# NVlabs/FoundationPose

Hardware: NVIDIA H100
Metric: pose-hypotheses/sec at 640x480 RGB-D, 252 hyp, 5 refine iters (higher is better)
Workload: dtype f16

## Files before the change

foundationpose_b200/csrc/fp_api_ops.cu:

```cuda
#include "../../include/fpose.h"
#include "fp_common.cuh"
#include "fp_attn.cuh"
#include "fp_crop.cuh"
#include "fp_gemm.cuh"

#include <vector>

namespace fp {
const char* get_last_error();
int prof_collect(int kind, double* total_ms, double* total_work, int* launches);
int pose_errors_launch(const float* pts, int P, const float* pred, int N, const float* gt, int n_gt, float* add_out,
                       float* adds_out, cudaStream_t stream);
int sym_pose_errors_launch(const float* pts, int P, const float* pred, int N, const float* gt, int n_gt, const float* sym,
                           int S, const float* K, int n_K, float* mssd_out, float* mspd_out, cudaStream_t stream);
}

static int check_device_ptr(const void* p, const char* what, const char* fn = "fp_pose_errors") {
  int dev = 0;
  FP_CUDA_OK(cudaGetDevice(&dev));
  cudaPointerAttributes a;
  const cudaError_t e = cudaPointerGetAttributes(&a, p);
  if (e != cudaSuccess) {
    cudaGetLastError();
    fp::set_last_error("%s: %s: cudaPointerGetAttributes failed (%s)", fn, what, cudaGetErrorString(e));
// ... 43 lines not shown
      }
    std::vector<float> nrm((size_t)V * 3, 0.f), att((size_t)V * 3, 0.f);
    fp::MeshHost mh;
    int rc = fp::build_mesh_host(V, F, pos, nrm.data(), att.data(), 3, faces, mh);
    if (rc) return rc;
    int max_t = 0, max_v = 0, total = 0;
    for (const fp::Meshlet& m : mh.meshlets) {
      max_t = m.n_tris > max_t ? m.n_tris : max_t;
      max_v = m.n_verts > max_v ? m.n_verts : max_v;
      total += m.n_tris;
      for (int t = 0; t < m.n_tris; ++t) {
        const uint2 tr = mh.ml_tris[m.tri_off + t];
        for (int k = 0; k < 3; ++k) {
          const int slot = (tr.x >> (8 * k)) & 255;
          if (slot >= m.n_verts || mh.ml_verts[m.vert_off + slot] != faces[3 * tr.y + k]) {
            fp::set_last_error("fp_op_build_meshlets: meshlet triangle does not map back to its face");
            return -4;
          }
          const float* q = pos + 3 * faces[3 * tr.y + k];
          const float dx = q[0] - m.cx, dy = q[1] - m.cy, dz = q[2] - m.cz;
          if (dx * dx + dy * dy + dz * dz > m.r * m.r * 1.0001f + 1e-12f) {
            fp::set_last_error("fp_op_build_meshlets: vertex outside the meshlet's bounding sphere");
            return -4;
          }
        }
        if (face_of_tri_out) face_of_tri_out[m.tri_off + t] = (int)tr.y;
      }
    }
    if (meshlets_out)
      for (size_t i = 0; i < mh.meshlets.size(); ++i) {
        const fp::Meshlet& m = mh.meshlets[i];
        const float rec[8] = {m.cx, m.cy, m.cz, m.r, m.ax, m.ay, m.az, m.cutoff};
        for (int k = 0; k < 8; ++k) meshlets_out[8 * i + k] = rec[k];
      }
    info[0] = (int)mh.meshlets.size();
    info[1] = mh.closed;
    info[2] = mh.front_sign;
    info[3] = max_t;
    info[4] = max_v;
    info[5] = total;
    return 0;
  } catch (...) {
    fp::set_last_error("fp_op_build_meshlets: exception");
    return -3;
  }
}

int fp_op_attention(const void* qkv, void* out, int B, int impl, void* stream) {
  if (!qkv || !out) {
    fp::set_last_error("fp_op_attention: null argument");
    return -1;
  }
  (void)impl;
  return fp::attn_tc_launch(
      fp::head_attn_params(reinterpret_cast<const __half*>(qkv), 1536, 1, reinterpret_cast<__half*>(out), B),
      reinterpret_cast<cudaStream_t>(stream));
}

static int check_dev16(const void* p, const char* what, const char* fn) {
  FP_REQUIRE(p, "%s: %s is null", fn, what);
  FP_REQUIRE(reinterpret_cast<uintptr_t>(p) % 16 == 0, "%s: %s is not 16-byte aligned", fn, what);
  return check_device_ptr(p, what, fn);
}

int fp_op_attention_groups(const void* qkv, int ld, int n_groups, void* out, int B, void* stream) {
  const char* fn = "fp_op_attention_groups";
  FP_REQUIRE(n_groups == 1 || n_groups == 2, "%s: n_groups = %d, must be 1 or 2", fn, n_groups);
  FP_REQUIRE(ld >= 1536 * n_groups && ld % 8 == 0, "%s: ld = %d, must be a multiple of 8 and >= %d", fn, ld, 1536 * n_groups);
  FP_REQUIRE(B >= 0 && B <= FP_OP_MAX_SEQUENCES, "%s: B = %d outside [0, %d]", fn, B, FP_OP_MAX_SEQUENCES);
  if (check_dev16(qkv, "qkv", fn) || check_dev16(out, "out", fn)) return -1;
  return fp::attn_core_launch(
      fp::head_attn_params(reinterpret_cast<const __half*>(qkv), ld, n_groups, reinterpret_cast<__half*>(out), B),
      reinterpret_cast<cudaStream_t>(stream));
}

int fp_op_layernorm(const void* x, void* y, const float* gamma, const float* beta, int rows, void* stream) {
  const char* fn = "fp_op_layernorm";
  FP_REQUIRE(rows >= 0 && rows <= FP_OP_MAX_SEQUENCES * 400, "%s: rows = %d outside [0, %d]", fn, rows,
             FP_OP_MAX_SEQUENCES * 400);
  if (check_dev16(x, "x", fn) || check_dev16(y, "y", fn) || check_dev16(gamma, "gamma", fn) || check_dev16(beta, "beta", fn))
    return -1;
  return fp::layernorm_launch(reinterpret_cast<const __half*>(x), reinterpret_cast<__half*>(y), gamma, beta, rows,
                              reinterpret_cast<cudaStream_t>(stream));
}

int fp_op_head_final(const void* x, const float* gamma, const float* beta, const float* w, const float* bias, float* out,
                     int B, int out_dim, void* stream) {
  const char* fn = "fp_op_head_final";
  FP_REQUIRE(B >= 0 && B <= FP_OP_MAX_SEQUENCES, "%s: B = %d outside [0, %d]", fn, B, FP_OP_MAX_SEQUENCES);
  FP_REQUIRE(out_dim >= 1 && out_dim <= 8, "%s: out_dim = %d outside [1, 8]", fn, out_dim);
  if (check_dev16(x, "x", fn) || check_dev16(gamma, "gamma", fn) || check_dev16(beta, "beta", fn)) return -1;
  FP_REQUIRE(w && bias && out, "%s: null w, bias or out", fn);
  if (check_device_ptr(w, "w", fn) || check_device_ptr(bias, "bias", fn) || check_device_ptr(out, "out", fn)) return -1;
  return fp::head_final_launch(reinterpret_cast<const __half*>(x), gamma, beta, w, bias, out, B, 400, out_dim,
                               reinterpret_cast<cudaStream_t>(stream));
}

int fp_op_token_mean_proj(const void* x, const float* w_f32, const float* bias, float* mean_ws, float* out, int B,
                          void* stream) {
  const char* fn = "fp_op_token_mean_proj";
  FP_REQUIRE(B >= 0 && B <= FP_OP_MAX_SEQUENCES, "%s: B = %d outside [0, %d]", fn, B, FP_OP_MAX_SEQUENCES);
  if (check_dev16(x, "x", fn) || check_dev16(w_f32, "w_f32", fn) || check_dev16(mean_ws, "mean_ws", fn)) return -1;
  FP_REQUIRE(bias && out, "%s: null bias or out", fn);
  if (check_device_ptr(bias, "bias", fn) || check_device_ptr(out, "out", fn)) return -1;
  return fp::token_mean_proj_launch(reinterpret_cast<const __half*>(x), w_f32, bias, mean_ws, out, B, 400,
                                    reinterpret_cast<cudaStream_t>(stream));
}

static fp::GemmLayer to_gemm_layer(const fp_gemm_layer_t* l) {
  fp::GemmLayer L;
  L.kind = l->kind;
  L.n_img = l->n_img;
  L.Hin = l->Hin;
  L.Win = l->Win;
  L.Cin = l->Cin;
  L.Cout = l->Cout;
  L.in = l->in;
  L.w = l->w;
  L.bias = l->bias;
  L.res = l->res;
  L.res_ld = l->res_ld;
  L.out = l->out;
  L.out_ld = l->out_ld;
  L.out_split = l->out_split;
  L.post_add = l->post_add;
  L.relu = l->relu;
  return L;
}

int fp_op_gemm_layer(const fp_gemm_layer_t* l, void* stream) {
  if (!l) {
    fp::set_last_error("fp_op_gemm_layer: null layer");
    return -1;
  }
  return fp::gemm_layer_launch(to_gemm_layer(l), reinterpret_cast<cudaStream_t>(stream));
}

int fp_op_gemm_tile_n(const fp_gemm_layer_t* l, int* tile_n) {
  if (!l || !tile_n) {
    fp::set_last_error("fp_op_gemm_tile_n: null argument");
    return -1;
  }
  return fp::gemm_layer_tile_n(to_gemm_layer(l), tile_n);
}

int fp_op_gemm_tile_m(const fp_gemm_layer_t* l, int* tile_m) {
  if (!l || !tile_m) {
    fp::set_last_error("fp_op_gemm_tile_m: null argument");
    return -1;
  }
  return fp::gemm_layer_tile_m(to_gemm_layer(l), tile_m);
}

int fp_pose_errors(const float* pts, int P, const float* pred, int N, const float* gt, int n_gt, float* add_out,
                   float* adds_out, void* stream) {
  FP_REQUIRE(P >= 1 && P <= FP_METRICS_MAX_POINTS, "fp_pose_errors: P = %d outside [1, %d]", P, FP_METRICS_MAX_POINTS);
  FP_REQUIRE(N >= 0 && N <= FP_METRICS_MAX_POSES, "fp_pose_errors: N = %d outside [0, %d]", N, FP_METRICS_MAX_POSES);
  FP_REQUIRE(n_gt == 1 || n_gt == N, "fp_pose_errors: n_gt = %d, must be 1 or N = %d", n_gt, N);
  if (N == 0) return 0;
  FP_REQUIRE(pts && pred && gt, "fp_pose_errors: null input pointer");
  const void* ptrs[5] = {pts, pred, gt, add_out, adds_out};
  const char* names[5] = {"pts", "pred", "gt", "add_out", "adds_out"};
  for (int i = 0; i < 5; ++i)
    if (ptrs[i] && check_device_ptr(ptrs[i], names[i])) return -1;
  return fp::pose_errors_launch(pts, P, pred, N, gt, n_gt, add_out, adds_out, reinterpret_cast<cudaStream_t>(stream));
}

int fp_sym_pose_errors(const float* pts, int P, const float* pred, int N, const float* gt, int n_gt, const float* sym,
                       int S, const float* K, int n_K, float* mssd_out, float* mspd_out, void* stream) {
  FP_REQUIRE(P >= 1 && P <= FP_METRICS_MAX_POINTS, "fp_sym_pose_errors: P = %d outside [1, %d]", P, FP_METRICS_MAX_POINTS);
  FP_REQUIRE(N >= 0 && N <= FP_METRICS_MAX_POSES, "fp_sym_pose_errors: N = %d outside [0, %d]", N, FP_METRICS_MAX_POSES);
  FP_REQUIRE(S >= 1 && S <= FP_METRICS_MAX_SYMMETRIES, "fp_sym_pose_errors: S = %d outside [1, %d]", S,
             FP_METRICS_MAX_SYMMETRIES);
  FP_REQUIRE(n_gt == 1 || n_gt == N, "fp_sym_pose_errors: n_gt = %d, must be 1 or N = %d", n_gt, N);
  if (mspd_out) FP_REQUIRE(n_K == 1 || n_K == N, "fp_sym_pose_errors: n_K = %d, must be 1 or N = %d", n_K, N);
  if (N == 0) return 0;
  FP_REQUIRE(pts && pred && gt && sym, "fp_sym_pose_errors: null input pointer");
  FP_REQUIRE(K || !mspd_out, "fp_sym_pose_errors: mspd_out needs K");
  const void* ptrs[7] = {pts, pred, gt, sym, mspd_out ? K : nullptr, mssd_out, mspd_out};
  const char* names[7] = {"pts", "pred", "gt", "sym", "K", "mssd_out", "mspd_out"};
  for (int i = 0; i < 7; ++i)
    if (ptrs[i] && check_device_ptr(ptrs[i], names[i], "fp_sym_pose_errors")) return -1;
  return fp::sym_pose_errors_launch(pts, P, pred, N, gt, n_gt, sym, S, K, n_K, mssd_out, mspd_out,
                                    reinterpret_cast<cudaStream_t>(stream));
}

}
```

foundationpose_b200/csrc/fp_gemm.cu:

```cuda
#include "fp_gemm.cuh"

#include <stdarg.h>
#include <stdlib.h>
#include <string.h>

#include <mutex>
#include <vector>

#include "fp_common.cuh"
#include "fp_wgmma.cuh"

namespace fp {

static std::atomic<unsigned long long> g_launch_count{0};
static thread_local bool t_capturing = false;
void note_launches(int n) {
  if (!t_capturing) g_launch_count.fetch_add((unsigned long long)n, std::memory_order_relaxed);
}
unsigned long long launch_count() { return g_launch_count.load(std::memory_order_relaxed); }
void set_capturing(bool on) { t_capturing = on; }

std::atomic<bool> g_prof_on{false};
static std::mutex g_prof_mu;

// ... 252 lines not shown
        mbar_arrive(&empty[prev]);
      }
      prev = stage;
      if (++stage == S) {
        stage = 0;
        phase ^= 1;
      }
    }
    if constexpr (kSwap) {
      const float bc[2] = {__ldg(p.bias + n_tile * BN + r0), __ldg(p.bias + n_tile * BN + r0 + 8)};
      wgmma_wait<0>();
      fence_regs(acc);
      if (prev >= 0) mbar_arrive(&empty[prev]);
      if (p.has_res) mbar_wait(&res_full[0], (uint32_t)(it & 1));
      else asm volatile("bar.sync 1, 256;" ::: "memory");
      const int mi = lane >> 3, mr = lane & 7;
      const uint32_t lane_off =
          (uint32_t)(8 * (mi >> 1) + mr) * 128u + ((uint32_t)((2 * ((ct >> 5) & 3) + (mi & 1)) ^ mr) << 4);
#pragma unroll
      for (int ph = 0; ph < 2; ++ph) {
        const uint32_t slab = smem_u32(staging + (2 * ph + cw) * kSlabBytes) + lane_off;
        uint32_t rv[8][4];
        if (p.has_res) {
#pragma unroll
          for (int g = 0; g < 8; ++g) ldsm_x4_trans(slab + g * 2048u, rv[g]);
        }
#pragma unroll
        for (int g = 0; g < 8; ++g) {
          uint32_t o[4];
#pragma unroll
          for (int i = 0; i < 4; ++i) {
            const int j = 16 * ph + 2 * g + (i >> 1), h = i & 1;
            float a0 = acc[4 * j + 2 * h] + bc[h], a1 = acc[4 * j + 2 * h + 1] + bc[h];
            if (p.has_res) {
              const float2 r = __half22float2(*reinterpret_cast<const __half2*>(&rv[g][i]));
              a0 += r.x;
              a1 += r.y;
            }
            if (p.relu) {
              a0 = fmaxf(a0, 0.f);
              a1 = fmaxf(a1, 0.f);
            }
            o[i] = pack_half2(a0, a1);
          }
          stsm_x4_trans(slab + g * 2048u, o);
        }
      }
      asm volatile("fence.proxy.async.shared::cta;" ::: "memory");
      asm volatile("bar.sync 1, 256;" ::: "memory");
      if (leader) {
        for (int q = 0; q < NSLAB; ++q)
          tma_store_5d(&map_out, staging + q * kSlabBytes, coff + n_tile * BN + slab_ch(q), oc[1], oc[2],
                       oc[3] + slab_img(q), oc[4]);
        asm volatile("cp.async.bulk.commit_group;" ::: "memory");
      }
      continue;
    }
    const float* bias = p.bias + n_tile * BN;
    const float* pap[2] = {nullptr, nullptr};
    if (p.post_add) {
#pragma unroll
      for (int h = 0; h < 2; ++h) {
        const int row = r0 + 8 * h;
        const int jj = row & (p.bw - 1), ii = (row >> p.lg_bw) & (p.bh - 1);
        const int i = th * p.bh + ii, j = min(tw * p.bw + jj, p.Wo - 1);
        pap[h] = p.post_add + (size_t)(i * p.Wo + j) * p.Cout + n_tile * BN;
      }
    }
    float2 pe[8][2];
    auto load_pe = [&](int b) {
#pragma unroll
      for (int jl = 0; jl < 8; ++jl)
#pragma unroll
        for (int h = 0; h < 2; ++h) pe[jl][h] = __ldg(reinterpret_cast<const float2*>(pap[h] + 64 * b + 8 * jl + cq));
    };
    if (p.post_add) load_pe(0);
    wgmma_wait<0>();
    fence_regs(acc);
    if (prev >= 0) mbar_arrive(&empty[prev]);
    if (!p.has_res) asm volatile("bar.sync 1, 256;" ::: "memory");

#pragma unroll
    for (int b = 0; b < NB; ++b) {
      const int s = kAlt ? (b & 1) : b;
      uint8_t* slab = staging + s * kSlabBytes;
      if (kAlt && p.has_res && b > 0 && b + 1 < NB) {
        if (leader) {
          asm volatile("cp.async.bulk.wait_group.read 0;" ::: "memory");
          uint64_t* rb = &res_full[(b + 1) & 1];
          mbar_expect_tx(rb, kSlabBytes);
          tma_load_5d(&map_res, rb, staging + ((b + 1) & 1) * kSlabBytes, n_tile * BN + (b + 1) * 64, rc[1], rc[2],
                      rc[3], rc[4]);
        }
      }
      if (p.has_res && (kAlt || b == 0))
        mbar_wait(&res_full[kAlt ? s : 0], (uint32_t)((it * (NB / NSLAB) + b / NSLAB) & 1));
#pragma unroll
      for (int jh = 0; jh < 8; jh += 4) {
        float2 bb[4];
        __half2 rv[4][2];
#pragma unroll
        for (int jl = 0; jl < 4; ++jl) {
          bb[jl] = __ldg(reinterpret_cast<const float2*>(bias + 64 * b + 8 * (jh + jl) + cq));
          if (p.has_res) {
#pragma unroll
            for (int h = 0; h < 2; ++h) {
              const int row = r0 + 8 * h;
              rv[jl][h] = *reinterpret_cast<const __half2*>(slab + row * 128 + (((uint32_t)(jh + jl) ^ (uint32_t)(row & 7)) << 4) + cq * 2);
            }
          }
        }
#pragma unroll
        for (int jl = 0; jl < 4; ++jl) {
          const int j = 8 * b + jh + jl;
#pragma unroll
          for (int h = 0; h < 2; ++h) {
            const int row = r0 + 8 * h;
            uint32_t* cell = reinterpret_cast<uint32_t*>(slab + row * 128 + (((uint32_t)(jh + jl) ^ (uint32_t)(row & 7)) << 4) + cq * 2);
            float a0 = acc[4 * j + 2 * h] + bb[jl].x, a1 = acc[4 * j + 2 * h + 1] + bb[jl].y;
            if (p.has_res) {
              const float2 r = __half22float2(rv[jl][h]);
              a0 += r.x;
              a1 += r.y;
            }
            if (p.relu) {
              a0 = fmaxf(a0, 0.f);
              a1 = fmaxf(a1, 0.f);
            }
            if (p.post_add) {
              a0 += pe[jh + jl][h].x;
              a1 += pe[jh + jl][h].y;
            }
            *cell = pack_half2(a0, a1);
          }
        }
      }
      if (p.post_add && b + 1 < NB) load_pe(b + 1);
      if (kAlt || b == NB - 1) {
        asm volatile("fence.proxy.async.shared::cta;" ::: "memory");
        if (kAlt && leader) asm volatile("cp.async.bulk.wait_group.read 0;" ::: "memory");
        asm volatile("bar.sync 1, 256;" ::: "memory");
        if (leader) {
          for (int q = kAlt ? s : 0; q < (kAlt ? s + 1 : NSLAB); ++q)
            tma_store_5d(&map_out, staging + q * kSlabBytes, coff + n_tile * BN + (kAlt ? 64 * b : 64 * q), oc[1],
                         oc[2], oc[3], oc[4]);
          asm volatile("cp.async.bulk.commit_group;" ::: "memory");
        }
      }
    }
  }
  if (leader) asm volatile("cp.async.bulk.wait_group 0;" ::: "memory");
}

static int g_num_sms = 0;

typedef CUresult (*EncodeTiledFn)(CUtensorMap*, CUtensorMapDataType, cuuint32_t, void*, const cuuint64_t*,
                                  const cuuint64_t*, const cuuint32_t*, const cuuint32_t*,
                                  CUtensorMapInterleave, CUtensorMapSwizzle, CUtensorMapL2promotion,
                                  CUtensorMapFloatOOBfill);

static EncodeTiledFn get_encode_fn() {
  static EncodeTiledFn fn = nullptr;
  static std::once_flag once;
  std::call_once(once, [] {
    void* p = nullptr;
    cudaDriverEntryPointQueryResult qres;
    if (cudaGetDriverEntryPoint("cuTensorMapEncodeTiled", &p, cudaEnableDefault, &qres) == cudaSuccess &&
        qres == cudaDriverEntryPointSuccess)
      fn = reinterpret_cast<EncodeTiledFn>(p);
  });
  return fn;
}

static int encode_map(CUtensorMap* map, const void* base, int rank, const uint64_t* dims,
                      const uint64_t* strides_bytes , const uint32_t* box, bool swizzle128 = true) {
  EncodeTiledFn fn = get_encode_fn();
  FP_REQUIRE(fn != nullptr, "cuTensorMapEncodeTiled entry point not available (no CUDA driver?)");
  cuuint64_t gdim[5];
  cuuint64_t gstr[4];
  cuuint32_t bdim[5];
  cuuint32_t estr[5];
  for (int i = 0; i < rank; ++i) {
    gdim[i] = dims[i];
    bdim[i] = box[i];
    estr[i] = 1;
  }
  for (int i = 0; i < rank - 1; ++i) gstr[i] = strides_bytes[i];
  CUresult r = fn(map, CU_TENSOR_MAP_DATA_TYPE_FLOAT16, (cuuint32_t)rank, const_cast<void*>(base), gdim, gstr,
                  bdim, estr, CU_TENSOR_MAP_INTERLEAVE_NONE, swizzle128 ? CU_TENSOR_MAP_SWIZZLE_128B : CU_TENSOR_MAP_SWIZZLE_NONE,
                  CU_TENSOR_MAP_L2_PROMOTION_L2_256B, CU_TENSOR_MAP_FLOAT_OOB_FILL_NONE);
  FP_REQUIRE(r == CUDA_SUCCESS,
             "cuTensorMapEncodeTiled failed (%d): rank %d dims [%llu %llu %llu %llu %llu] box [%u %u %u %u %u]",
             (int)r, rank, (unsigned long long)dims[0], (unsigned long long)(rank > 1 ? dims[1] : 0),
             (unsigned long long)(rank > 2 ? dims[2] : 0), (unsigned long long)(rank > 3 ? dims[3] : 0),
             (unsigned long long)(rank > 4 ? dims[4] : 0), box[0], rank > 1 ? box[1] : 0, rank > 2 ? box[2] : 0,
             rank > 3 ? box[3] : 0, rank > 4 ? box[4] : 0);
  return 0;
}

int encode_map_f16(CUtensorMap* map, const void* base, int rank, const uint64_t* dims, const uint64_t* strides_bytes,
                   const uint32_t* box) {
  return encode_map(map, base, rank, dims, strides_bytes, box);
}
int encode_map_f16_linear(CUtensorMap* map, const void* base, int rank, const uint64_t* dims,
                          const uint64_t* strides_bytes, const uint32_t* box) {
  return encode_map(map, base, rank, dims, strides_bytes, box, false);
}
int num_sms() {
  if (g_num_sms == 0) {
    int dev = 0;
    if (cudaGetDevice(&dev) != cudaSuccess) return 0;
    if (cudaDeviceGetAttribute(&g_num_sms, cudaDevAttrMultiProcessorCount, dev) != cudaSuccess) return 0;
  }
  return g_num_sms;
}

static int ilog2(int v) {
  int l = 0;
  while ((1 << l) < v) ++l;
  return l;
}

template <int BN, bool kSwap = false>
static int launch_bn(const CUtensorMap& ma, const CUtensorMap& mb, const CUtensorMap& mo, const CUtensorMap& mr,
                     const GemmParams& p, cudaStream_t stream) {
  using Cfg = TileCfg<BN, kSwap>;
  static std::atomic<unsigned long long> attr_mask{0};
  if (!device_bit_test(attr_mask)) {
    FP_CUDA_OK(cudaFuncSetAttribute(gemm_tile_kernel<BN, kSwap>, cudaFuncAttributeMaxDynamicSharedMemorySize,
                                    Cfg::kSmemBytes));
    device_bit_set(attr_mask);
  }
  const int sms = num_sms();
  FP_REQUIRE(sms > 0, "no CUDA device");
  const int grid = p.total_tiles < sms ? p.total_tiles : sms;
  prof_mark_begin(0, p.alg_flops, stream);
  FP_CUDA_OK(launch_pdl(gemm_tile_kernel<BN, kSwap>, dim3(grid), dim3(kTileThreads), Cfg::kSmemBytes, stream, 1, ma, mb,
                        mo, mr, p));
  prof_mark_end(stream);
  note_launches(1);
  FP_CUDA_OK(cudaGetLastError());
  return 0;
}

int stem_conv_launch(const GemmLayer& L, cudaStream_t stream);

static bool swap_tile_enabled() {
  const char* e = getenv("FPOSE_SWAP_TILE");
  return !(e && e[0] == '0');
}

static int gemm_layer_plan(const GemmLayer& L, cudaStream_t stream, int* tile_n, int* tile_m) {
  if (L.kind == LK_CONV7_S2) {
    if (tile_n || tile_m) {
      if (tile_n) *tile_n = 64;
      if (tile_m) *tile_m = 128;
      return 0;
    }
    return stem_conv_launch(L, stream);
  }
  GemmParams p;
  memset(&p, 0, sizeof(p));
  CUtensorMap ma, mb;
  const uint64_t E = 2;
  int Ho, Wo, taps, ktot;
  int BN;
  uint64_t dims[5], str[4];
  uint32_t box[5];

  switch (L.kind) {
    case LK_LINEAR: {
      FP_REQUIRE(L.Cin % 64 == 0, "LINEAR: K=%d not a multiple of 64", L.Cin);
      Ho = 1;
      Wo = L.Win;
      taps = 1;
      p.chunks_per_tap = L.Cin / 64;
      p.bw = 128; p.bh = 1; p.bn = 1;
      p.dim_w = 1; p.dim_h = -1; p.dim_n = -1;
      dims[0] = L.Cin; dims[1] = L.Win; dims[2] = 1; dims[3] = 1; dims[4] = 1;
      str[0] = L.Cin * E; str[1] = str[0] * L.Win; str[2] = str[1]; str[3] = str[1];
      box[0] = 64; box[1] = 128; box[2] = 1; box[3] = 1; box[4] = 1;
      p.tiles_w = (L.Win + 127) / 128; p.tiles_h = 1; p.tiles_n = 1;
      break;
    }
    case LK_CONV3_S1: {
      FP_REQUIRE(L.Cin % 64 == 0, "CONV3_S1: Cin=%d not a multiple of 64", L.Cin);
      Ho = L.Hin; Wo = L.Win;
      taps = 9;
      p.chunks_per_tap = L.Cin / 64;
      if (Wo % 8 == 0 && Ho % 8 == 0) { p.bw = 8; p.bh = 8; p.bn = 2; }
      else if (Wo % 4 == 0 && Ho % 4 == 0) { p.bw = 4; p.bh = 4; p.bn = 8; }
      else FP_REQUIRE(false, "CONV3_S1: unsupported spatial size %dx%d", Ho, Wo);
      const uint64_t sw_ = (uint64_t)L.Cin * E, sh_ = sw_ * L.Win, sn_ = sh_ * L.Hin;
      p.dim_w = 1; p.dim_h = 2; p.dim_n = 3;
      dims[0] = L.Cin; dims[1] = L.Win; dims[2] = L.Hin; dims[3] = L.n_img; dims[4] = 1;
      str[0] = sw_; str[1] = sh_; str[2] = sn_; str[3] = sn_ * L.n_img;
      box[0] = 64; box[1] = p.bw; box[2] = p.bh; box[3] = p.bn; box[4] = 1;
      for (int r = 0; r < 3; ++r)
        for (int s = 0; s < 3; ++s) {
          p.tap_off[r * 3 + s][1] = (short)(s - 1);
          p.tap_off[r * 3 + s][2] = (short)(r - 1);
        }
      p.tiles_w = Wo / p.bw; p.tiles_h = Ho / p.bh; p.tiles_n = (L.n_img + p.bn - 1) / p.bn;
      break;
    }
    case LK_CONV3_S2: {
      FP_REQUIRE(L.Cin % 64 == 0, "CONV3_S2: Cin=%d not a multiple of 64", L.Cin);
      FP_REQUIRE(L.Hin % 2 == 0 && L.Win % 2 == 0, "CONV3_S2: odd input size");
      Ho = L.Hin / 2; Wo = L.Win / 2;
      taps = 9;
      p.chunks_per_tap = L.Cin / 64;
      if (Wo % 8 == 0 && Ho % 8 == 0) { p.bw = 8; p.bh = 8; p.bn = 2; }
      else if (Wo % 4 == 0 && Ho % 4 == 0) { p.bw = 4; p.bh = 4; p.bn = 8; }
      else FP_REQUIRE(false, "CONV3_S2: unsupported output size %dx%d", Ho, Wo);
      p.dim_w = 1; p.dim_h = 3; p.dim_n = 4;
      dims[0] = 2 * L.Cin; dims[1] = Wo; dims[2] = 2; dims[3] = Ho; dims[4] = L.n_img;
      str[0] = 2 * L.Cin * E; str[1] = (uint64_t)L.Win * L.Cin * E; str[2] = 2 * str[1];
      str[3] = (uint64_t)L.Hin * L.Win * L.Cin * E;
      box[0] = 64; box[1] = p.bw; box[2] = 1; box[3] = p.bh; box[4] = p.bn;
      for (int r = 0; r < 3; ++r)
        for (int s = 0; s < 3; ++s) {
          const int t = r * 3 + s;
          p.tap_off[t][0] = (short)((s == 1 ? 0 : 1) * L.Cin);
          p.tap_off[t][1] = (short)(s == 0 ? -1 : 0);
          p.tap_off[t][2] = (short)(r == 1 ? 0 : 1);
          p.tap_off[t][3] = (short)(r == 0 ? -1 : 0);
        }
      p.tiles_w = Wo / p.bw; p.tiles_h = Ho / p.bh; p.tiles_n = (L.n_img + p.bn - 1) / p.bn;
      break;
    }
    default:
      FP_REQUIRE(false, "unknown layer kind %d", L.kind);
  }
  ktot = taps * L.Cin;
  p.num_kb = ktot / 64;
  p.lg_bw = ilog2(p.bw);
  p.lg_bh = ilog2(p.bh);

  constexpr int kWideMinWaves = 8;
  constexpr int kWideMinKBlocks = 16;
  bool swap = false;
  if (L.Cout == 128 && L.kind != LK_LINEAR && p.bw == 8 && p.num_kb >= kWideMinKBlocks && !L.post_add &&
      L.out_split % 4 == 0 && swap_tile_enabled()) {
    const int sms = num_sms();
    FP_REQUIRE(sms > 0, "no CUDA device");
    swap = (long long)p.tiles_w * p.tiles_h * ((L.n_img + 3) / 4) >= (long long)kWideMinWaves * sms;
  }
  if (swap) {
    p.bn = 4;
    box[p.dim_n] = 4;
    p.tiles_n = (L.n_img + 3) / 4;
  }
  const int m_tiles = p.tiles_w * p.tiles_h * p.tiles_n;
  if (swap) BN = 128;
  else if (L.Cout % 256 == 0 && p.num_kb >= kWideMinKBlocks) {
    const int sms = num_sms();
    FP_REQUIRE(sms > 0, "no CUDA device");
    BN = (long long)m_tiles * (L.Cout / 256) >= (long long)kWideMinWaves * sms ? 256 : 128;
  } else if (L.Cout % 128 == 0) BN = 128;
  else if (L.Cout % 64 == 0) BN = 64;
  else FP_REQUIRE(false, "Cout=%d must be a multiple of 64", L.Cout);
  p.n_tiles_n = L.Cout / BN;
  p.total_tiles = p.tiles_w * p.tiles_h * p.tiles_n * p.n_tiles_n;
  p.Ho = Ho; p.Wo = Wo; p.n_img = L.n_img; p.Cout = L.Cout;
  p.bias = L.bias;
  p.has_res = L.res != nullptr;
  p.out_split = L.out_split;
  p.post_add = L.post_add;
  p.relu = L.relu;
  {
    const double k_real = (double)taps * L.Cin;
    p.alg_flops = 2.0 * (double)L.n_img * Ho * Wo * L.Cout * k_real;
  }
  FP_REQUIRE(L.out_ld % 8 == 0 && (!L.res || L.res_ld % 8 == 0), "out_ld / res_ld must be multiples of 8");
  FP_REQUIRE(L.out_split == 0 || L.out_split % p.bn == 0,
             "out_split=%d must be a multiple of the tile's image count %d (pad the A/B batch boundary)", L.out_split,
             p.bn);
  if (tile_n || tile_m) {
    if (tile_n) *tile_n = BN;
    if (tile_m) *tile_m = swap ? 256 : 128;
    return 0;
  }
  if (p.total_tiles == 0) return 0;

  int rc = encode_map(&ma, L.in, 5, dims, str, box);
  if (rc) return rc;
  uint64_t wd[2] = {(uint64_t)ktot, (uint64_t)L.Cout};
  uint64_t ws[1] = {(uint64_t)ktot * E};
  uint32_t wb[2] = {64, (uint32_t)BN};
  rc = encode_map(&mb, L.w, 2, wd, ws, wb);
  if (rc) return rc;
  CUtensorMap mo, mr;
  {
    uint64_t od[5], os[4];
    uint32_t ob[5];
    const bool lin = (L.kind == LK_LINEAR);
    const int n_out = L.out_split > 0 ? (L.n_img - L.out_split) : L.n_img;
    FP_REQUIRE(n_out > 0, "out_split=%d leaves no output images (n_img=%d)", L.out_split, L.n_img);
    auto fill = [&](int ld, int nimg) {
      const uint64_t sw_ = (uint64_t)ld * E, sh_ = sw_ * Wo, sn_ = sh_ * Ho;
      od[0] = (uint64_t)ld;
      ob[0] = 64;
      od[4] = 1;
      ob[4] = 1;
      if (lin) {
        od[1] = (uint64_t)Wo; od[2] = 1; od[3] = 1;
        os[0] = sw_; os[1] = sh_; os[2] = sh_; os[3] = sh_;
        ob[1] = (uint32_t)p.bw; ob[2] = 1; ob[3] = 1;
      } else {
        od[1] = (uint64_t)Wo; od[2] = (uint64_t)Ho; od[3] = (uint64_t)nimg;
        os[0] = sw_; os[1] = sh_; os[2] = sn_; os[3] = sn_ * nimg;
        ob[1] = (uint32_t)p.bw; ob[2] = (uint32_t)p.bh; ob[3] = (uint32_t)(swap ? p.bn / 2 : p.bn);
      }
    };
    p.odim_h = lin ? -1 : 2;
    p.odim_n = lin ? -1 : 3;
    fill(L.out_ld, n_out);
    rc = encode_map(&mo, L.out, 5, od, os, ob);
    if (rc) return rc;
    if (L.res) {
      fill(L.res_ld, L.n_img);
      rc = encode_map(&mr, L.res, 5, od, os, ob);
      if (rc) return rc;
    } else {
      mr = mo;
    }
  }
  if (swap) return launch_bn<128, true>(ma, mb, mo, mr, p, stream);
  if (BN == 256) return launch_bn<256>(ma, mb, mo, mr, p, stream);
  return BN == 128 ? launch_bn<128>(ma, mb, mo, mr, p, stream) : launch_bn<64>(ma, mb, mo, mr, p, stream);
}

int gemm_layer_launch(const GemmLayer& L, cudaStream_t stream) { return gemm_layer_plan(L, stream, nullptr, nullptr); }

int gemm_layer_tile_n(const GemmLayer& L, int* tile_n) { return gemm_layer_plan(L, nullptr, tile_n, nullptr); }

int gemm_layer_tile_m(const GemmLayer& L, int* tile_m) { return gemm_layer_plan(L, nullptr, nullptr, tile_m); }

}
```

foundationpose_b200/csrc/fp_gemm.cuh:

```cuda
#pragma once
#include <cuda.h>
#include <cuda_runtime.h>
#include <stdint.h>

#include <atomic>

namespace fp {

enum LayerKind : int {
  LK_LINEAR = 0,
  LK_CONV3_S1 = 1,
  LK_CONV3_S2 = 2,
  LK_CONV7_S2 = 3,
};

struct GemmLayer {
  int kind;
  int n_img;
  int Hin, Win;
  int Cin;
  int Cout;
  const void* in;
  const void* w;
  const float* bias;
  const void* res;
  int res_ld;
  void* out;
  int out_ld;
  int out_split;
  const float* post_add;
  int relu;
};

int gemm_layer_launch(const GemmLayer& L, cudaStream_t stream);
int gemm_layer_tile_n(const GemmLayer& L, int* tile_n);
int gemm_layer_tile_m(const GemmLayer& L, int* tile_m);


void prof_mark_begin(int kind, double work, cudaStream_t stream);
void prof_mark_end(cudaStream_t stream);
extern std::atomic<bool> g_prof_on;

}
```

foundationpose_b200/ops.py:

```python
import ctypes as C

import torch

from . import _lib
from ._lib import lib


def _ptr(t):
    return None if t is None else C.c_void_p(t.data_ptr())


def _stream():
    return C.c_void_p(torch.cuda.current_stream().cuda_stream)


def _require_cuda(*ts):
    for t in ts:
        if t is not None and not t.is_cuda:
            raise _lib.FposeError("libfpose operators need CUDA tensors (there is no CPU path)")


def gemm_layer(kind, x, w_packed, bias, *, n_img, Hin, Win, Cin, Cout, out=None, out_ld=None, out_split=0,
               res=None, res_ld=0, post_add=None, relu=False):
    _require_cuda(x, w_packed, bias, res, post_add, out)
    assert x.dtype == torch.float16 and w_packed.dtype == torch.float16 and bias.dtype == torch.float32
    if kind == _lib.LAYER_LINEAR:
        Ho, Wo = 1, Win
    elif kind == _lib.LAYER_CONV3_S1:
        Ho, Wo = Hin, Win
    else:
        Ho, Wo = Hin // 2, Win // 2
    if out is None:
        out_ld = Cout
        out = torch.empty(n_img, Ho, Wo, Cout, dtype=torch.float16, device=x.device)
    L = _lib.GemmLayer(kind, n_img, Hin, Win, Cin, Cout, _ptr(x), _ptr(w_packed), _ptr(bias), _ptr(res),
                       res_ld, _ptr(out), out_ld, out_split, _ptr(post_add), 1 if relu else 0)
    _lib.check(lib.fp_op_gemm_layer(C.byref(L), _stream()), "fp_op_gemm_layer")
    return out


def gemm_tile_n(kind, *, n_img, Hin, Win, Cin, Cout, out_split=0):
    lib.fp_op_gemm_tile_n.argtypes = [C.POINTER(_lib.GemmLayer), C.POINTER(C.c_int)]
    lib.fp_op_gemm_tile_n.restype = C.c_int
    L = _lib.GemmLayer(kind, n_img, Hin, Win, Cin, Cout, None, None, None, None, 0, None, Cout, out_split, None, 0)
    tile_n = C.c_int(0)
    _lib.check(lib.fp_op_gemm_tile_n(C.byref(L), C.byref(tile_n)), "fp_op_gemm_tile_n")
    return tile_n.value


def gemm_tile_m(kind, *, n_img, Hin, Win, Cin, Cout, out_split=0):
    lib.fp_op_gemm_tile_m.argtypes = [C.POINTER(_lib.GemmLayer), C.POINTER(C.c_int)]
    lib.fp_op_gemm_tile_m.restype = C.c_int
    L = _lib.GemmLayer(kind, n_img, Hin, Win, Cin, Cout, None, None, None, None, 0, None, Cout, out_split, None, 0)
    tile_m = C.c_int(0)
    _lib.check(lib.fp_op_gemm_tile_m(C.byref(L), C.byref(tile_m)), "fp_op_gemm_tile_m")
    return tile_m.value


lib.fp_op_attention.argtypes = [C.c_void_p, C.c_void_p, C.c_int, C.c_int, C.c_void_p]
lib.fp_op_attention.restype = C.c_int


def attention(qkv, impl=1):
    _require_cuda(qkv)
    assert qkv.dtype == torch.float16 and qkv.shape[1] == 1536 and qkv.shape[0] % 400 == 0
    B = qkv.shape[0] // 400
    out = torch.empty(qkv.shape[0], 512, dtype=torch.float16, device=qkv.device)
    _lib.check(lib.fp_op_attention(_ptr(qkv), _ptr(out), B, impl, _stream()), "fp_op_attention")
    return out


lib.fp_op_attention_groups.argtypes = [C.c_void_p, C.c_int, C.c_int, C.c_void_p, C.c_int, C.c_void_p]
lib.fp_op_attention_groups.restype = C.c_int
lib.fp_op_layernorm.argtypes = [C.c_void_p, C.c_void_p, C.c_void_p, C.c_void_p, C.c_int, C.c_void_p]
lib.fp_op_layernorm.restype = C.c_int
lib.fp_op_head_final.argtypes = [C.c_void_p] * 6 + [C.c_int, C.c_int, C.c_void_p]
lib.fp_op_head_final.restype = C.c_int
lib.fp_op_token_mean_proj.argtypes = [C.c_void_p] * 5 + [C.c_int, C.c_void_p]
lib.fp_op_token_mean_proj.restype = C.c_int


def attention_groups(qkv, B, n_groups, *, ld=None):
    _require_cuda(qkv)
    assert qkv.dtype == torch.float16 and qkv.stride(-1) == 1
    ld = qkv.stride(0) if ld is None else ld
    out = torch.empty(n_groups, B * 400, 512, dtype=torch.float16, device=qkv.device)
    _lib.check(lib.fp_op_attention_groups(_ptr(qkv), ld, n_groups, _ptr(out), B, _stream()), "fp_op_attention_groups")
    return out


def layernorm(x, gamma, beta):
    _require_cuda(x, gamma, beta)
    assert x.dtype == torch.float16 and x.is_contiguous() and x.shape[-1] == 512
    assert gamma.dtype == torch.float32 and beta.dtype == torch.float32
    y = torch.empty_like(x)
    rows = x.numel() // 512
    _lib.check(lib.fp_op_layernorm(_ptr(x), _ptr(y), _ptr(gamma), _ptr(beta), rows, _stream()), "fp_op_layernorm")
    return y


def head_final(x, gamma, beta, w, bias):
    _require_cuda(x, gamma, beta, w, bias)
    assert x.dtype == torch.float16 and x.is_contiguous() and x.shape[1:] == (400, 512)
    B, out_dim = x.shape[0], w.shape[0]
    out = torch.empty(B, out_dim, dtype=torch.float32, device=x.device)
    _lib.check(lib.fp_op_head_final(_ptr(x), _ptr(gamma), _ptr(beta), _ptr(w.contiguous()), _ptr(bias), _ptr(out), B, out_dim,
                                    _stream()), "fp_op_head_final")
    return out


def token_mean_proj(x, w, bias):
    _require_cuda(x, w, bias)
    assert x.dtype == torch.float16 and x.is_contiguous() and x.shape[1:] == (400, 512)
    assert w.dtype == torch.float32 and w.is_contiguous() and w.shape == (512, 512)
    B = x.shape[0]
    mean_ws = torch.empty(B, 512, dtype=torch.float32, device=x.device)
    out = torch.empty(B, 512, dtype=torch.float32, device=x.device)
    _lib.check(lib.fp_op_token_mean_proj(_ptr(x), _ptr(w), _ptr(bias), _ptr(mean_ws), _ptr(out), B, _stream()),
               "fp_op_token_mean_proj")
    return out
```

include/fpose.h:

```cpp
#ifndef FPOSE_H_
#define FPOSE_H_

#include <stddef.h>
#include <stdint.h>

#ifdef __cplusplus
extern "C" {
#endif

const char* fp_last_error(void);
unsigned long long fp_launch_count(void);

int fp_prof_enable(int on);
int fp_prof_collect(int kind, double* total_ms, double* total_work, int* launches);


#define FP_LAYER_LINEAR 0
#define FP_LAYER_CONV3_S1 1
#define FP_LAYER_CONV3_S2 2
#define FP_LAYER_CONV7_S2 3

typedef struct fp_gemm_layer {
  int kind;
  int n_img;
  int Hin, Win;
  int Cin;
  int Cout;
  const void* in;
  const void* w;
  const float* bias;
  const void* res;
  int res_ld;
  void* out;
  int out_ld;
  int out_split;
  const float* post_add;
  int relu;
} fp_gemm_layer_t;

int fp_op_gemm_layer(const fp_gemm_layer_t* layer, void* stream);
int fp_op_gemm_tile_n(const fp_gemm_layer_t* layer, int* tile_n);
int fp_op_gemm_tile_m(const fp_gemm_layer_t* layer, int* tile_m);

int fp_op_attention(const void* qkv, void* out, int B, int impl, void* stream);

#define FP_OP_MAX_SEQUENCES 65536
int fp_op_attention_groups(const void* qkv, int ld, int n_groups, void* out, int B, void* stream);
int fp_op_layernorm(const void* x, void* y, const float* gamma, const float* beta, int rows, void* stream);
int fp_op_head_final(const void* x, const float* gamma, const float* beta, const float* w, const float* bias, float* out,
                     int B, int out_dim, void* stream);
int fp_op_token_mean_proj(const void* x, const float* w_f32, const float* bias, float* mean_ws, float* out, int B,
                          void* stream);



#define FP_METRICS_MAX_POINTS 131072
#define FP_METRICS_MAX_POSES (1 << 24)
int fp_pose_errors(const float* pts, int P, const float* pred, int N, const float* gt, int n_gt,
                   float* add_out, float* adds_out, void* stream);

#define FP_METRICS_MAX_SYMMETRIES 4096
int fp_sym_pose_errors(const float* pts, int P, const float* pred, int N, const float* gt, int n_gt, const float* sym,
                       int S, const float* K, int n_K, float* mssd_out, float* mspd_out, void* stream);

typedef struct fp_ctx fp_ctx;

int fp_create(fp_ctx** ctx);
int fp_destroy(fp_ctx* ctx);

int fp_set_config(fp_ctx* ctx, int which, float crop_ratio, float rot_normalizer);

typedef struct fp_tensor {
  const char* name;
  const void* data;
  int dtype;
  long long numel;
} fp_tensor_t;

int fp_load_network(fp_ctx* ctx, int which, const fp_tensor_t* tensors, int n);

int fp_set_mesh(fp_ctx* ctx, int V, int F, const float* pos, const float* nrm, const float* uv, const float* vcol,
                const int* faces, const unsigned char* tex_rgb, int Ht, int Wt, float diameter);
#define FP_MAX_MESHES 64
int fp_set_mesh_slot(fp_ctx* ctx, int slot, int V, int F, const float* pos, const float* nrm, const float* uv,
                     const float* vcol, const int* faces, const unsigned char* tex_rgb, int Ht, int Wt, float diameter);
int fp_mesh_info(fp_ctx* ctx, int* info);

#define FP_FRAME_ON_DEVICE 1
#define FP_FRAME_FILTER_DEPTH 2
int fp_set_frame(fp_ctx* ctx, const unsigned char* rgb, const float* depth, const float* K, int H, int W, int flags,
                 float zfar, void* stream);
int fp_set_xyz_map(fp_ctx* ctx, const float* xyz, void* stream);
int fp_get_depth(fp_ctx* ctx, float* depth_out_dev, float* xyz_out_dev, void* stream);

int fp_start_poses(fp_ctx* ctx, const unsigned char* mask, int mask_on_device, const float* rot_grid, int N,
                   float* poses_out, float* info_out, void* stream);

int fp_make_crops(fp_ctx* ctx, const float* poses, int N, int mode, void* crops_out, float* dbg_out, float* win_out,
                  void* stream);
int fp_set_crop_tile(fp_ctx* ctx, int tile);
int fp_crop_stats(fp_ctx* ctx, const float* poses, int N, int mode, int* stats_out_host, void* stream);

int fp_refine(fp_ctx* ctx, const float* poses_in, int N, int iterations, float* poses_out, float* last_trans,
              float* last_rot, void* stream);

int fp_score(fp_ctx* ctx, const float* poses, int N, float* scores_out, int* best_out, void* stream);
int fp_score_features(fp_ctx* ctx, const float* poses, int N, float* feats_out, void* stream);
int fp_score_tail(fp_ctx* ctx, const float* feats, int L, float* scores_out, int* best_out, void* stream);

int fp_register(fp_ctx* ctx, const float* poses_host, int N, int iterations, float* poses_out_host,
                float* scores_out_host, int* best_out_host, void* stream);

int fp_track(fp_ctx* ctx, const unsigned char* rgb_host, const float* depth_host, const float* K, int H, int W,
             const float* pose_in_dev, int iterations, float* pose_out_dev, float* pose_out_host, void* stream);
int fp_track_objects(fp_ctx* ctx, const unsigned char* rgb_host, const float* depth_host, const float* K, int H, int W,
                     int M, const int* slots_host, const float* poses_in_dev, int iterations, float* poses_out_dev,
                     float* poses_out_host, void* stream);
#define FP_MAX_CAMERAS 16
int fp_track_cameras(fp_ctx* ctx, int C, const unsigned char* const* rgb_host, const float* const* depth_host,
                     const float* K, const int* H, const int* W, int M, const int* camera_of, const int* slots_host,
                     const float* poses_in_dev, int iterations, float* poses_out_dev, float* poses_out_host, void* stream);
int fp_register_objects(fp_ctx* ctx, const unsigned char* rgb_host, const float* depth_host, const float* K, int H, int W,
                        int M, const int* slots_host, const int* n_hyp_host, const unsigned char* masks_host,
                        const float* rot_grids_dev, int iterations, float* poses_out_dev, float* scores_out_dev,
                        int* best_out_dev, float* info_out_dev, void* stream);
int fp_register_cameras(fp_ctx* ctx, int C, const unsigned char* const* rgb_host, const float* const* depth_host,
                        const float* K, const int* H, const int* W, int M, const int* camera_of, const int* slots_host,
                        const int* n_hyp_host, const unsigned char* const* masks_host, const float* rot_grids_dev,
                        int iterations, float* poses_out_dev, float* scores_out_dev, int* best_out_dev, float* info_out_dev,
                        void* stream);
unsigned long long fp_graph_captures(fp_ctx* ctx);

int fp_vis(fp_ctx* ctx, int kind, const float* poses_a, const float* poses_b, int N, const int* order,
           unsigned char* canvas_out, int* hw_out, void* stream);
int fp_vis_size(int kind, int N, int* hw_out);
int fp_vis_colormap(unsigned char* rgb_out);
int fp_vis_crops(fp_ctx* ctx, const float* poses, int N, int mode, float* rec_out, void* stream);
unsigned long long fp_vis_workspace_bytes(fp_ctx* ctx);

typedef struct fp_group fp_group;
int fp_group_create(int ndev, const int* dev_ids, fp_group** out);
int fp_group_destroy(fp_group* g);
int fp_group_size(fp_group* g);
fp_ctx* fp_group_ctx(fp_group* g, int i);
int fp_group_load_network(fp_group* g, int which, const fp_tensor_t* tensors, int n);
int fp_group_set_config(fp_group* g, int which, float crop_ratio, float rot_normalizer);
int fp_group_set_mesh(fp_group* g, int V, int F, const float* pos, const float* nrm, const float* uv, const float* vcol,
                      const int* faces, const unsigned char* tex_rgb, int Ht, int Wt, float diameter);
int fp_group_register(fp_group* g, const unsigned char* rgb_host, const float* depth_host, const float* K, int H, int W,
                      const unsigned char* mask_host, const float* rot_grid_host, int N, int iterations,
                      float* poses_out_host, float* scores_out_host, int* best_out_host, float* info_out_host);

int fp_op_refine_net(fp_ctx* ctx, const void* crops, int N, float* trans_out, float* rot_out, void* stream);
int fp_op_score_feats(fp_ctx* ctx, const void* crops, int N, float* feats_out, void* stream);
int fp_op_tokens(fp_ctx* ctx, int which, const void* crops, int N, void* tokens_out, void* stream);
int fp_op_build_meshlets(int V, int F, const float* pos, const int* faces, int* info, int* face_of_tri_out,
                         float* meshlets_out );
int fp_op_depth_filter(const float* depth_dev, float* out_dev, int H, int W, int which, void* stream);
int fp_op_pose_update(const float* poses_in, const float* trans, const float* rot, float* poses_out, int N,
                      float mesh_diameter, float rot_normalizer, void* stream);

#ifdef __cplusplus
}
#endif
#endif
```

Before: 3739.

## Add ping-pong warpgroup GEMM kernel for K=512 linear layers

Adds a persistent GEMM kernel where two consumer warpgroups alternate tiles, ordered by named barriers, so one warpgroup's epilogue (bias, residual, relu, TMA store) overlaps the other's WGMMA main loop. A single producer thread feeds a shared TMA ring of stages. The kernel is selected for linear layers with Cin=512, BN=128, no post_add or out_split, and enough tiles to fill several waves, and can be disabled through an environment variable. It also exposes a query for whether a layer uses the ping-pong path. The cost is a second accumulator set per warpgroup and more complex synchronisation that could hurt small grids.

```diff
diff --git a/foundationpose_b200/csrc/fp_api_ops.cu b/foundationpose_b200/csrc/fp_api_ops.cu
--- a/foundationpose_b200/csrc/fp_api_ops.cu
+++ b/foundationpose_b200/csrc/fp_api_ops.cu
@@ -219,6 +219,14 @@
   return fp::gemm_layer_tile_m(to_gemm_layer(l), tile_m);
 }
 
+int fp_op_gemm_pingpong(const fp_gemm_layer_t* l, int* pingpong) {
+  if (!l || !pingpong) {
+    fp::set_last_error("fp_op_gemm_pingpong: null argument");
+    return -1;
+  }
+  return fp::gemm_layer_pingpong(to_gemm_layer(l), pingpong);
+}
+
 int fp_pose_errors(const float* pts, int P, const float* pred, int N, const float* gt, int n_gt, float* add_out,
                    float* adds_out, void* stream) {
   FP_REQUIRE(P >= 1 && P <= FP_METRICS_MAX_POINTS, "fp_pose_errors: P = %d outside [1, %d]", P, FP_METRICS_MAX_POINTS);
diff --git a/foundationpose_b200/csrc/fp_gemm.cu b/foundationpose_b200/csrc/fp_gemm.cu
--- a/foundationpose_b200/csrc/fp_gemm.cu
+++ b/foundationpose_b200/csrc/fp_gemm.cu
@@ -428,6 +428,181 @@
   if (leader) asm volatile("cp.async.bulk.wait_group 0;" ::: "memory");
 }
 
+struct PingPongCfg {
+  static constexpr int kBBytes = 128 * kBlockK * 2;
+  static constexpr int kStageBytes = kABytes + kBBytes;
+  static constexpr int kSlabs = 2;
+  static constexpr int kStagingBytes = 2 * kSlabs * kSlabBytes;
+  static constexpr int kStages = (kSmemOptIn - kStagingBytes - 1024  - 256 ) / kStageBytes;
+  static constexpr int kSmemBytes = kStages * kStageBytes + kStagingBytes + 1024 + 256;
+  static_assert(kStages >= 4, "the ring must hold half of a tile's eight k-blocks");
+  static_assert(kSmemBytes <= kSmemOptIn, "tile configuration exceeds the 227 KB opt-in shared memory");
+  static_assert((2 * kStages + 2) * 8 <= 256, "the mbarriers must fit their 256 bytes");
+};
+
+__global__ void __launch_bounds__(kTileThreads, 1)
+    gemm_pingpong_kernel(const __grid_constant__ CUtensorMap map_a, const __grid_constant__ CUtensorMap map_b,
+                         const __grid_constant__ CUtensorMap map_out, const __grid_constant__ CUtensorMap map_res,
+                         const __grid_constant__ GemmParams p) {
+  using Cfg = PingPongCfg;
+  constexpr int S = Cfg::kStages;
+  extern __shared__ uint8_t smem_raw[];
+  uint8_t* smem = smem_raw + ((1024u - (smem_u32(smem_raw) & 1023u)) & 1023u);
+  uint8_t* staging = smem + S * Cfg::kStageBytes;
+  uint64_t* bars = reinterpret_cast<uint64_t*>(staging + Cfg::kStagingBytes);
+  uint64_t* full = bars;
+  uint64_t* empty = bars + S;
+  uint64_t* res_full = bars + 2 * S;
+
+  const int total = p.tiles_w * p.n_tiles_n;
+
+  if (threadIdx.x == 0) {
+    tma_prefetch_desc(&map_a);
+    tma_prefetch_desc(&map_b);
+    tma_prefetch_desc(&map_out);
+    if (p.has_res) tma_prefetch_desc(&map_res);
+    for (int s = 0; s < S; ++s) {
+      mbar_init(&full[s], 1);
+      mbar_init(&empty[s], 128);
+    }
+    for (int w = 0; w < 2; ++w) mbar_init(&res_full[w], 1);
+    mbar_fence_init();
+  }
+  __syncthreads();
+  pdl_trigger();
+  pdl_wait();
+
+  if (threadIdx.x < 128) {
+    regs_release<kWideProducerRegs>();
+    if (threadIdx.x == 0) {
+      int stage = 0, phase = 0;
+      for (int t = blockIdx.x; t < total; t += gridDim.x) {
+        const int n_tile = t % p.n_tiles_n, tw = t / p.n_tiles_n;
+        for (int kb = 0; kb < p.num_kb; ++kb) {
+          mbar_wait(&empty[stage], phase ^ 1);
+          uint8_t* sa = smem + stage * Cfg::kStageBytes;
+          mbar_expect_tx(&full[stage], Cfg::kStageBytes);
+          tma_load_5d(&map_a, &full[stage], sa, kb * kBlockK, tw * 128, 0, 0, 0);
+          tma_load_2d(&map_b, &full[stage], sa + kABytes, kb * kBlockK, n_tile * 128);
+          if (++stage == S) {
+            stage = 0;
+            phase ^= 1;
+          }
+        }
+      }
+    }
+    return;
+  }
+
+  regs_acquire<kWideConsumerRegs>();
+  const int ct = threadIdx.x - 128;
+  const int cw = ct >> 7;
+  const int wt = ct & 127;
+  const int lane = threadIdx.x & 31;
+  const int r0 = 16 * (wt >> 5) + (lane >> 2);
+  const int cq = 2 * (lane & 3);
+  const bool leader = (wt == 0);
+  uint8_t* slabs = staging + cw * Cfg::kSlabs * kSlabBytes;
+  uint64_t* rbar = &res_full[cw];
+  const uint32_t epi_bar = 1 + cw;
+  float acc[2][64];
+  int it = 0;
+  for (int i = cw; blockIdx.x + i * gridDim.x < total; i += 2, ++it) {
+    const int t = blockIdx.x + i * gridDim.x;
+    const int n_tile = t % p.n_tiles_n, tw = t / p.n_tiles_n;
+    if (i > 0) asm volatile("bar.sync %0, 256;" ::"r"(3 + (i & 1)) : "memory");
+    int g = i * p.num_kb;
+    int prev = -1;
+    for (int kb = 0; kb < p.num_kb; ++kb, ++g) {
+      const int stage = g % S;
+      mbar_wait(&full[stage], (uint32_t)((g / S) & 1));
+      const uint32_t sa = smem_u32(smem + stage * Cfg::kStageBytes);
+      const uint64_t db = gmma_desc_sw128(sa + kABytes);
+      wgmma_fence();
+#pragma unroll
+      for (int k = 0; k < kBlockK / 16; ++k)
+#pragma unroll
+        for (int h = 0; h < 2; ++h)
+          Wgmma<128>::ss(acc[h], gmma_desc_sw128(sa + (uint32_t)h * 8192u) + (uint64_t)(2 * k), db + (uint64_t)(2 * k),
+                         (kb > 0 || k > 0) ? 1u : 0u);
+      wgmma_commit();
+      if (kb == 0 && leader) {
+        asm volatile("cp.async.bulk.wait_group.read 0;" ::: "memory");
+        if (p.has_res) {
+          mbar_expect_tx(rbar, Cfg::kSlabs * kSlabBytes);
+          for (int s = 0; s < Cfg::kSlabs; ++s)
+            tma_load_5d(&map_res, rbar, slabs + s * kSlabBytes, n_tile * 128 + 64 * s, tw * 128, 0, 0, 0);
+        }
+      }
+      if (prev >= 0) {
+        wgmma_wait<1>();
+        mbar_arrive(&empty[prev]);
+      }
+      prev = stage;
+    }
+    if (blockIdx.x + (i + 1) * gridDim.x < total) asm volatile("bar.arrive %0, 256;" ::"r"(3 + ((i + 1) & 1)) : "memory");
+
+    const float* bias = p.bias + n_tile * 128;
+    wgmma_wait<0>();
+    fence_regs(acc[0]);
+    fence_regs(acc[1]);
+    mbar_arrive(&empty[prev]);
+    if (p.has_res) mbar_wait(rbar, (uint32_t)(it & 1));
+    else asm volatile("bar.sync %0, 128;" ::"r"(epi_bar) : "memory");
+#pragma unroll
+    for (int b = 0; b < 2; ++b) {
+      uint8_t* slab = slabs + b * kSlabBytes;
+#pragma unroll
+      for (int jh = 0; jh < 8; jh += 4) {
+        float2 bb[4];
+#pragma unroll
+        for (int jl = 0; jl < 4; ++jl) bb[jl] = __ldg(reinterpret_cast<const float2*>(bias + 64 * b + 8 * (jh + jl) + cq));
+#pragma unroll
+        for (int hm = 0; hm < 2; ++hm) {
+          __half2 rv[4][2];
+          if (p.has_res) {
+#pragma unroll
+            for (int jl = 0; jl < 4; ++jl)
+#pragma unroll
+              for (int h = 0; h < 2; ++h) {
+                const int row = 64 * hm + r0 + 8 * h;
+                rv[jl][h] = *reinterpret_cast<const __half2*>(slab + row * 128 + (((uint32_t)(jh + jl) ^ (uint32_t)(row & 7)) << 4) + cq * 2);
+              }
+          }
+#pragma unroll
+          for (int jl = 0; jl < 4; ++jl) {
+            const int j = 8 * b + jh + jl;
+#pragma unroll
+            for (int h = 0; h < 2; ++h) {
+              const int row = 64 * hm + r0 + 8 * h;
+              uint32_t* cell = reinterpret_cast<uint32_t*>(slab + row * 128 + (((uint32_t)(jh + jl) ^ (uint32_t)(row & 7)) << 4) + cq * 2);
+              float a0 = acc[hm][4 * j + 2 * h] + bb[jl].x, a1 = acc[hm][4 * j + 2 * h + 1] + bb[jl].y;
+              if (p.has_res) {
+                const float2 r = __half22float2(rv[jl][h]);
+                a0 += r.x;
+                a1 += r.y;
+              }
+              if (p.relu) {
+                a0 = fmaxf(a0, 0.f);
+                a1 = fmaxf(a1, 0.f);
+              }
+              *cell = pack_half2(a0, a1);
+            }
+          }
+        }
+      }
+    }
+    asm volatile("fence.proxy.async.shared::cta;" ::: "memory");
+    asm volatile("bar.sync %0, 128;" ::"r"(epi_bar) : "memory");
+    if (leader) {
+      for (int q = 0; q < Cfg::kSlabs; ++q)
+        tma_store_5d(&map_out, slabs + q * kSlabBytes, n_tile * 128 + 64 * q, tw * 128, 0, 0, 0);
+      asm volatile("cp.async.bulk.commit_group;" ::: "memory");
+    }
+  }
+  if (leader) asm volatile("cp.async.bulk.wait_group 0;" ::: "memory");
+}
+
 static int g_num_sms = 0;
 
 typedef CUresult (*EncodeTiledFn)(CUtensorMap*, CUtensorMapDataType, cuuint32_t, void*, const cuuint64_t*,
@@ -525,12 +700,38 @@
   const char* e = getenv("FPOSE_SWAP_TILE");
   return !(e && e[0] == '0');
 }
-
-static int gemm_layer_plan(const GemmLayer& L, cudaStream_t stream, int* tile_n, int* tile_m) {
+static bool pingpong_tile_enabled() {
+  const char* e = getenv("FPOSE_PINGPONG_TILE");
+  return !(e && e[0] == '0');
+}
+
+static int launch_pingpong(const CUtensorMap& ma, const CUtensorMap& mb, const CUtensorMap& mo, const CUtensorMap& mr,
+                           const GemmParams& p, cudaStream_t stream) {
+  static std::atomic<unsigned long long> attr_mask{0};
+  if (!device_bit_test(attr_mask)) {
+    FP_CUDA_OK(cudaFuncSetAttribute(gemm_pingpong_kernel, cudaFuncAttributeMaxDynamicSharedMemorySize,
+                                    PingPongCfg::kSmemBytes));
+    device_bit_set(attr_mask);
+  }
+  const int sms = num_sms();
+  FP_REQUIRE(sms > 0, "no CUDA device");
+  const int grid = p.total_tiles < sms ? p.total_tiles : sms;
+  prof_mark_begin(0, p.alg_flops, stream);
+  FP_CUDA_OK(launch_pdl(gemm_pingpong_kernel, dim3(grid), dim3(kTileThreads), PingPongCfg::kSmemBytes, stream, 1, ma, mb,
+                        mo, mr, p));
+  prof_mark_end(stream);
+  note_launches(1);
+  FP_CUDA_OK(cudaGetLastError());
+  return 0;
+}
+
+static int gemm_layer_plan(const GemmLayer& L, cudaStream_t stream, int* tile_n, int* tile_m, int* pingpong) {
+  const bool query = tile_n || tile_m || pingpong;
   if (L.kind == LK_CONV7_S2) {
-    if (tile_n || tile_m) {
+    if (query) {
       if (tile_n) *tile_n = 64;
       if (tile_m) *tile_m = 128;
+      if (pingpong) *pingpong = 0;
       return 0;
     }
     return stem_conv_launch(L, stream);
@@ -638,6 +839,12 @@
   else FP_REQUIRE(false, "Cout=%d must be a multiple of 64", L.Cout);
   p.n_tiles_n = L.Cout / BN;
   p.total_tiles = p.tiles_w * p.tiles_h * p.tiles_n * p.n_tiles_n;
+  bool pp = false;
+  if (L.kind == LK_LINEAR && L.Cin == 512 && BN == 128 && !L.post_add && L.out_split == 0 && pingpong_tile_enabled()) {
+    const int sms = num_sms();
+    FP_REQUIRE(sms > 0, "no CUDA device");
+    pp = (long long)p.total_tiles >= (long long)kWideMinWaves * sms;
+  }
   p.Ho = Ho; p.Wo = Wo; p.n_img = L.n_img; p.Cout = L.Cout;
   p.bias = L.bias;
   p.has_res = L.res != nullptr;
@@ -652,9 +859,10 @@
   FP_REQUIRE(L.out_split == 0 || L.out_split % p.bn == 0,
              "out_split=%d must be a multiple of the tile's image count %d (pad the A/B batch boundary)", L.out_split,
              p.bn);
-  if (tile_n || tile_m) {
+  if (query) {
     if (tile_n) *tile_n = BN;
     if (tile_m) *tile_m = swap ? 256 : 128;
+    if (pingpong) *pingpong = pp ? 1 : 0;
     return 0;
   }
   if (p.total_tiles == 0) return 0;
@@ -702,15 +910,22 @@
       mr = mo;
     }
   }
+  if (pp) return launch_pingpong(ma, mb, mo, mr, p, stream);
   if (swap) return launch_bn<128, true>(ma, mb, mo, mr, p, stream);
   if (BN == 256) return launch_bn<256>(ma, mb, mo, mr, p, stream);
   return BN == 128 ? launch_bn<128>(ma, mb, mo, mr, p, stream) : launch_bn<64>(ma, mb, mo, mr, p, stream);
 }
 
-int gemm_layer_launch(const GemmLayer& L, cudaStream_t stream) { return gemm_layer_plan(L, stream, nullptr, nullptr); }
-
-int gemm_layer_tile_n(const GemmLayer& L, int* tile_n) { return gemm_layer_plan(L, nullptr, tile_n, nullptr); }
-
-int gemm_layer_tile_m(const GemmLayer& L, int* tile_m) { return gemm_layer_plan(L, nullptr, nullptr, tile_m); }
-
-}
+int gemm_layer_launch(const GemmLayer& L, cudaStream_t stream) {
+  return gemm_layer_plan(L, stream, nullptr, nullptr, nullptr);
+}
+
+int gemm_layer_tile_n(const GemmLayer& L, int* tile_n) { return gemm_layer_plan(L, nullptr, tile_n, nullptr, nullptr); }
+
+int gemm_layer_tile_m(const GemmLayer& L, int* tile_m) { return gemm_layer_plan(L, nullptr, nullptr, tile_m, nullptr); }
+
+int gemm_layer_pingpong(const GemmLayer& L, int* pingpong) {
+  return gemm_layer_plan(L, nullptr, nullptr, nullptr, pingpong);
+}
+
+}
diff --git a/foundationpose_b200/csrc/fp_gemm.cuh b/foundationpose_b200/csrc/fp_gemm.cuh
--- a/foundationpose_b200/csrc/fp_gemm.cuh
+++ b/foundationpose_b200/csrc/fp_gemm.cuh
@@ -35,6 +35,7 @@
 int gemm_layer_launch(const GemmLayer& L, cudaStream_t stream);
 int gemm_layer_tile_n(const GemmLayer& L, int* tile_n);
 int gemm_layer_tile_m(const GemmLayer& L, int* tile_m);
+int gemm_layer_pingpong(const GemmLayer& L, int* pingpong);
 
 
 void prof_mark_begin(int kind, double work, cudaStream_t stream);
diff --git a/foundationpose_b200/ops.py b/foundationpose_b200/ops.py
--- a/foundationpose_b200/ops.py
+++ b/foundationpose_b200/ops.py
@@ -55,6 +55,15 @@
     tile_m = C.c_int(0)
     _lib.check(lib.fp_op_gemm_tile_m(C.byref(L), C.byref(tile_m)), "fp_op_gemm_tile_m")
     return tile_m.value
+
+
+def gemm_pingpong(kind, *, n_img, Hin, Win, Cin, Cout, out_split=0):
+    lib.fp_op_gemm_pingpong.argtypes = [C.POINTER(_lib.GemmLayer), C.POINTER(C.c_int)]
+    lib.fp_op_gemm_pingpong.restype = C.c_int
+    L = _lib.GemmLayer(kind, n_img, Hin, Win, Cin, Cout, None, None, None, None, 0, None, Cout, out_split, None, 0)
+    pingpong = C.c_int(0)
+    _lib.check(lib.fp_op_gemm_pingpong(C.byref(L), C.byref(pingpong)), "fp_op_gemm_pingpong")
+    return bool(pingpong.value)
 
 
 lib.fp_op_attention.argtypes = [C.c_void_p, C.c_void_p, C.c_int, C.c_int, C.c_void_p]
diff --git a/include/fpose.h b/include/fpose.h
--- a/include/fpose.h
+++ b/include/fpose.h
@@ -41,6 +41,7 @@
 int fp_op_gemm_layer(const fp_gemm_layer_t* layer, void* stream);
 int fp_op_gemm_tile_n(const fp_gemm_layer_t* layer, int* tile_n);
 int fp_op_gemm_tile_m(const fp_gemm_layer_t* layer, int* tile_m);
+int fp_op_gemm_pingpong(const fp_gemm_layer_t* layer, int* pingpong);
 
 int fp_op_attention(const void* qkv, void* out, int B, int impl, void* stream);
 
```

Result: faster. 3807 (median of 6 runs) (+1.8%).
